# Atif-Anwer/SHMGAN

Hardware: AMD Instinct MI355X
Metric: images/sec (gen+disc train_step) (higher is better)
Workload: dtype f32; 1 GPU; SHMGAN train_step 256x256 5-view, batch 8/GPU, filter_size 64, fp32 (BASELINE configs[1]); global_batch=8, image_size=256, parallelism=dp1, losses_finite=True

## Files before the change

### include/shmgan_hip.h

```cpp
#ifndef SHMGAN_HIP_H
#define SHMGAN_HIP_H

#include <stddef.h>

#ifdef __cplusplus
extern "C" {
#endif

#define SHM_OK 0
#define SHM_E_SHAPE (-1)
#define SHM_E_DTYPE (-2)
#define SHM_E_WORKSPACE (-3)
#define SHM_E_HIP (-4)

#define SHM_F32 0
#define SHM_BF16 1
#define SHM_BF16_GF32 2

int shm_version(void);
const char* shm_last_error(void);
const char* shm_last_kernel(void);

#define SHM_TG_AUTO 0
#define SHM_TG_HALO128 1
#define SHM_TG_HALO64 2
#define SHM_TG_DMA_128x128 3
#define SHM_TG_DMA_64x128 4
#define SHM_TG_DMA_128x64 5
#define SHM_TG_DMA_256x64 6
#define SHM_TG_DMA_256x128 7
#define SHM_TG_HALO128_PH8 8
#define SHM_TG_DMA_128x128_BK32 9
#define SHM_TG_DMA_128x128_NST4 10
#define SHM_TG_HALO128_ST 12
#define SHM_TG_HALO64_ST 13
#define SHM_TG_PHASE4 14
#define SHM_TG_DMA_64x64 15
#define SHM_TG_HALO128_ST_W4 16
#define SHM_TG_WREG 11
int shm_set_tuning(const char* key, int value);
int shm_get_tuning(const char* key, int* value);

int shm_transpose_taps(const float* w, void* wt, int ntaps, int rows, int cols, int rows_pad,
                       int dtype, void* stream);
int shm_transpose_taps_multi(int count, const void* const* w, void* const* wt, const int* ntaps, const int* rows,
                             const int* cols, const int* rows_pad, int dtype, void* stream);
int shm_cast_f32(const float* src, void* dst, size_t n, int dtype, void* stream);

int shm_conv2d_fwd(const void* x, const void* x2, int c1, int ldx, int ldx2, const void* wk,
                   const float* bias, void* y, int ldy, int batch, int hi, int wi, int cin,
                   int cout, int ksize, int stride, float slope, int dtype, void* stream);

#define SHM_STATS_SLOTS 16
int shm_conv2d_in_fwd(const void* x, const void* x2, int c1, int ldx, int ldx2, const void* wk,
                      const float* bias, void* y, int ldy, int batch, int hi, int wi, int cin,
                      int cout, int ksize, int stride, float slope, double* stats, double* scratch,
                      float eps, int dtype, void* stream);

int shm_conv2d_dgrad(const void* dy, int lddy, const void* w, void* dx, void* dx2, int n1,
                     int lddx, int lddx2, int batch, int hi, int wi, int cin, int cout,
                     int ksize, int stride, int dtype, void* stream);
// ... 219 lines not shown
```

### shmgan_amd/_lib.py

```python
from __future__ import annotations

import ctypes as C
import os
import re
import subprocess
from pathlib import Path

_HERE = Path(__file__).resolve().parent
LIB_PATH = Path(os.environ["SHM_LIB_PATH"]) if os.environ.get("SHM_LIB_PATH") else _HERE / "libshmgan_hip.so"
CSRC = _HERE / "csrc"
HEADER = _HERE.parent / "include" / "shmgan_hip.h"
SOURCES = ["runtime.hip", "conv_igemm.hip", "conv_dma.hip", "conv_halo.hip", "conv_wreg.hip", "conv_wreg_f32.hip", "conv_phase4.hip", "conv_wreg16.hip", "conv_pingpong.hip", "conv_wgrad.hip", "conv_wgrad_gen.hip", "conv_wgrad_halo.hip", "conv_wgrad_halo16.hip", "conv_wgrad_halo8.hip", "conv_wgrad_x3.hip", "conv_fwd_x3.hip", "conv_rgb.hip", "elem.hip", "instnorm.hip", "instnorm_bwd.hip", "instnorm_bwd_2pass.hip", "instnorm_bwd_fused8.hip", "instnorm_bwd_fusedg.hip", "grad_sums.hip", "heads.hip", "dgrad_sum1.hip", "color.hip", "imgloss.hip", "metrics.hip", "specseg.hip", "data.hip", "polar.hip", "export.hip", "telemetry.hip"]
SHARED_HEADERS = [CSRC / "common.h", CSRC / "elem.h", CSRC / "ablate.h", CSRC / "tapgemm.h", CSRC / "tapgemm_dev.h", CSRC / "wgrad.h", CSRC / "in_bwd.h", CSRC / "x3split.h", HEADER]
F32, BF16 = 0, 1
HIPCC_FLAGS = ["--offload-arch=gfx950", "-O3", "-fPIC", "-shared", "-munsafe-fp-atomics",
               "-Wall", "-Wno-unused-function", "-Wno-unused-local-typedef"]

EXTRA_FLAGS = {"conv_pingpong.hip": ["-fno-slp-vectorize"]}

P, I, Z, F = C.c_void_p, C.c_int, C.c_size_t, C.c_float

SIGNATURES = {
    "shm_version": (I, []),
    "shm_last_error": (C.c_char_p, []),
    "shm_last_kernel": (C.c_char_p, []),
    "shm_set_tuning": (I, [C.c_char_p, I]),
    "shm_get_tuning": (I, [C.c_char_p, P]),
    "shm_transpose_taps": (I, [P, P, I, I, I, I, I, P]),
    "shm_transpose_taps_multi": (I, [I, P, P, P, P, P, P, I, P]),
    "shm_cast_f32": (I, [P, P, Z, I, P]),
    "shm_conv2d_fwd": (I, [P, P, I, I, I, P, P, P, I, I, I, I, I, I, I, I, F, I, P]),
    "shm_conv2d_in_fwd": (I, [P, P, I, I, I, P, P, P, I, I, I, I, I, I, I, I, F, P, P, F, I, P]),
    "shm_conv2d_dgrad": (I, [P, I, P, P, P, I, I, I, I, I, I, I, I, I, I, I, P]),
    "shm_conv2d_transpose_fwd": (I, [P, I, P, P, P, I, I, I, I, I, I, F, I, P]),
    "shm_conv2d_wgrad_workspace": (Z, [I, I, I, I, I, I]),
# ... 151 lines not shown
```

### shmgan_amd/csrc/common.h

```cpp
#pragma once
#include <hip/hip_runtime.h>
#include <stddef.h>
#include <stdint.h>
#include <stdio.h>

#include "../../include/shmgan_hip.h"

typedef float f32x4 __attribute__((ext_vector_type(4)));
typedef float f32x16 __attribute__((ext_vector_type(16)));

typedef __bf16 bf16_t;

void shm_set_error(const char* fmt, ...);
void shm_set_last_kernel(const char* fmt, ...);

int shm_rgb_s2_fwd_launch(const void* x, int ldx, const void* wk, int K, const float* bias, void* y, int ldy, int batch, int hi, int wi, int cout, float slope,
                          double* stats, int stats_slots, unsigned stats_stride, size_t xbytes, size_t ybytes, int dtype, hipStream_t st);
int shm_rgb_s2_wgrad_launch(const void* x, int ldx, const void* dy, int lddy, float* part, size_t ws_bytes, int batch, int hi, int wi, int cin, int cout,
                            size_t xbytes, size_t dybytes, int dtype, int* nsplit_out, hipStream_t st);

int shm_in_finalize_internal(double* stats, double* part, int nslot, int total, int hw, double eps, float* nt, const float* beta, int c, hipStream_t st);
int shm_gsum_reduce_internal(const void* g, int ldg, const void* aux, int ldaux, double* red, int batch, int hw, int c, int dtype, hipStream_t st);

enum ShmTune {
// ... 2 lines not shown
    SHM_TUNE_TAPGEMM_SMALL_GRID,
    SHM_TUNE_TAPGEMM_PHASE4_MIN,
    SHM_TUNE_WGRAD_VARIANT,
    SHM_TUNE_WGRAD_BLOCKS,
    SHM_TUNE_WGRAD_BF16_ROWS,
    SHM_TUNE_STATS_FUSION,
    SHM_TUNE_ELEM_REVERSE,
    SHM_TUNE_ELEM_REDUCE_BLOCKS,
    SHM_TUNE_ELEM_NT,
    SHM_TUNE_ELEM_CHUNK_MB,
    SHM_TUNE_ELEM_INTERLEAVE,
    SHM_TUNE_ELEM_STREAM_BLOCKS,
    SHM_TUNE_ELEM_APPLY_BLOCKS,
    SHM_TUNE_TAPGEMM_WREG16,
    SHM_TUNE_WGRAD_BF16_WIDE,
    SHM_TUNE_WGRAD_F32_SPLIT,
    SHM_TUNE_TAPGEMM_FLAT_EPILOGUE,
    SHM_TUNE_ELEM_FUSED_BWD,
    SHM_TUNE_ELEM_FUSED_MAX_SLICES,
    SHM_TUNE_CONV_F32_SPLIT,
    SHM_TUNE_ELEM_FUSED_TEST_STALL,
    SHM_TUNE_ELEM_FUSED_HOLD,
    SHM_TUNE_ELEM_FUSED_GVARIANT,
    SHM_TUNE_COUNT
};
int shm_tune(int id);
unsigned long long* shm_clock_probe();

#define SHM_LDS_BARRIER()                                       \
    do {                                                        \
        asm volatile("s_waitcnt lgkmcnt(0)" ::: "memory");      \
        __builtin_amdgcn_s_barrier();                           \
    } while (0)

typedef unsigned shm_u32x4 __attribute__((ext_vector_type(4)));
__device__ __forceinline__ shm_u32x4 shm_rsrc_words(const void* p, unsigned bytes) {
    const unsigned long long a = (unsigned long long)p;
    return shm_u32x4{(unsigned)a, (unsigned)(a >> 32) & 0xffffu, bytes, 0x00020000u};
}
__device__ __forceinline__ void shm_dma16(const shm_u32x4 rs, const unsigned lds_addr, const unsigned voff) {
    unsigned keep;
    asm volatile("s_mov_b32 %0, m0\n\ts_mov_b32 m0, %1\n\ts_nop 0\n\tbuffer_load_dwordx4 %2, %3, 0 offen lds\n\ts_mov_b32 m0, %0"
                 : "=&s"(keep)
                 : "s"(lds_addr), "v"(voff), "s"(rs)
                 : "memory");
}
__device__ __forceinline__ unsigned shm_lds_addr(const void* p) {
    return (unsigned)(size_t)(__attribute__((address_space(3))) const void*)p;
}

#define SHM_TG_COUNT 17

__device__ __forceinline__ f32x4 ld4(const float* p) { return *(const f32x4*)p; }
__device__ __forceinline__ f32x4 ld4(const bf16_t* p) {
    const uint2 u = *(const uint2*)p;
    f32x4 r;
    r[0] = __uint_as_float(u.x << 16);
    r[1] = __uint_as_float(u.x & 0xffff0000u);
    r[2] = __uint_as_float(u.y << 16);
    r[3] = __uint_as_float(u.y & 0xffff0000u);
    return r;
}
__device__ __forceinline__ f32x4 ld4nt(const float* p) { return __builtin_nontemporal_load((const f32x4*)p); }
__device__ __forceinline__ f32x4 ld4nt(const bf16_t* p) {
    typedef unsigned u32x2_t __attribute__((ext_vector_type(2)));
    const u32x2_t u = __builtin_nontemporal_load((const u32x2_t*)p);
    f32x4 r;
    r[0] = __uint_as_float(u[0] << 16);
    r[1] = __uint_as_float(u[0] & 0xffff0000u);
    r[2] = __uint_as_float(u[1] << 16);
    r[3] = __uint_as_float(u[1] & 0xffff0000u);
    return r;
}
__device__ __forceinline__ void st4(float* p, f32x4 v) { *(f32x4*)p = v; }
// ... 121 lines not shown
```

### shmgan_amd/csrc/conv_halo.hip

```cpp
#include "tapgemm_dev.h"

template <typename T, typename TO, int BN, int PH = 16, bool ST = false, int TM = 2, bool GS = false, int NM = 0>
__global__ __launch_bounds__(BN * PH / (2 * TM), ST ? BN * PH / (256 * TM) : 1) void tapgemm_halo_kernel(const TapGemmArgs a) {
    static_assert(TM == 2 || (TM == 4 && ST), "four M tiles per wave: static-tap form only");
    static_assert(!NM || (ST && TM == 2 && !GS), "norm: static-tap forward form");
    constexpr int ESZ = sizeof(T), CHE = 16 / ESZ, BKE = 64 / ESZ;
    constexpr int WGM = PH / (2 * TM), WGN = BN / 64, NW = WGM * WGN;
    constexpr int HC = 18, NIT = PH == 16 ? 24 : 12;
    constexpr int NHR = NIT * 16;
    constexpr int ASTG = NHR * 16, BSTG = BN * 16;
    constexpr int NA = NIT / NW, NB = (BN / 16) / NW;
    static_assert(NIT % NW == 0 && (BN / 16) % NW == 0, "DMA items divide over the waves");
    __shared__ __attribute__((aligned(1024))) float smem[2 * ASTG + 3 * BSTG];
    __shared__ __attribute__((aligned(1024))) float snt[NM ? SHM_NT_PLANES * SHM_NT_MAXC : 4];
    float* const sA = smem;
    float* const sB = smem + 2 * ASTG;
    typedef __attribute__((address_space(3))) void* lds_ptr;

    const TapPhase& P = a.ph[0];
    const int tid = threadIdx.x;
    const int lane = tid & 63, wave = __builtin_amdgcn_readfirstlane(tid >> 6);
    const int l31 = lane & 31, h = lane >> 5;
    const int wm = wave / WGN, wn = wave % WGN;
    const int ppr = a.wi >> 4, ppi = (a.hi / PH) * ppr;
// ... 458 lines not shown
            const int py = 2 * TM * wm + 2 * i + (row >> 4), px = row & 15;
            const size_t opix = ((size_t)img * a.hi + (y0 + py)) * a.wi + (x0 + px);
#pragma unroll
            for (int j = 0; j < 2; ++j) {
                const int n = n0 + wn * 64 + j * 32 + l31;
                if (n < a.nout) {
                    float v = acc[i][j][r] + bj[j];
                    const TO vo = (TO)shm_lrelu(v, a.slope);
                    v = (float)vo;
                    s1[j] += v;
                    s2[j] = __builtin_fmaf(v, v, s2[j]);
                    if (!abl::nostore || v == 123.456f)
                    {
                        if (n < a.n1)
                            ((TO*)a.y)[opix * a.ldy + n] = vo;
                        else
                            ((TO*)a.y2)[opix * a.ldy2 + (n - a.n1)] = vo;
                    }
                }
            }
        }
    }
    }
    if (a.stats) {
        const int slot = (prem * WGM + wm) % a.stats_slots;
#pragma unroll
        for (int j = 0; j < 2; ++j) {
            float t1 = s1[j] + __shfl_xor(s1[j], 32, 64);
            float t2 = s2[j] + __shfl_xor(s2[j], 32, 64);
            const int n = n0 + wn * 64 + j * 32 + l31;
            if (h == 0 && n < a.nout) {
                double* dst = a.stats + (size_t)slot * a.stats_stride + ((size_t)img * a.nout + n) * 2;
                atomicAdd(dst, (double)t1);
                atomicAdd(dst + 1, (double)t2);
            }
        }
    }
}

template <typename T, typename TO, int BN, int PH = 16, bool ST = false, int TM = 2, bool GS = false, int NM = 0>
static void halo_launch(const TapGemmArgs& a, int batch, hipStream_t st) {
    hipLaunchKernelGGL((tapgemm_halo_kernel<T, TO, BN, PH, ST, TM, GS, NM>), dim3(batch * (a.hi / PH) * (a.wi / 16), shm_cdiv(a.nout, BN), 1), dim3(BN * PH / (2 * TM)), 0, st, a);
    shm_set_last_kernel("tapgemm_halo_kernel<%s, %s, %d, %d, %s, %d%s>", shm_tg_name<T>(), shm_tg_name<TO>(), BN, PH, ST ? "true" : "false", TM,
                        NM == 2 ? ", false, 2" : NM == 1 ? ", false, 1" : GS ? ", true" : "");
}

template <typename T, typename TO, int BN>
static void halo_st_launch(const TapGemmArgs& a, const TapGemmPlan& p, int batch, hipStream_t st) {
    if (p.gs_fused)
        halo_launch<T, TO, BN, 16, true, 2, true>(a, batch, st);
    else if (a.nt) {
        if constexpr (sizeof(T) == sizeof(TO)) {
            if (a.ntmode)
                halo_launch<T, TO, BN, 16, true, 2, false, 2>(a, batch, st);
            else
                halo_launch<T, TO, BN, 16, true, 2, false, 1>(a, batch, st);
        }
    } else
        halo_launch<T, TO, BN, 16, true>(a, batch, st);
}
// ... 27 lines not shown
```

### shmgan_amd/csrc/conv_igemm.hip

```cpp
#include "tapgemm.h"

struct ConvExtras {
    double* stats = nullptr;
    int stats_hw = 0, stats_slots = 1;
    const void* gaux[2] = {};
    int ldgaux[2] = {};
    double* gred[2] = {};
    ShmNormReq norm = {};
    bool gsum_fused = false;
};

static TapGemmPlan tapgemm_plan(const TapGemmArgs& a, int batch, int nphase, int esz, int oesz, bool two_src, bool want_norm) {
    const int BKE = 64 / esz;
    const int forced = shm_tune(SHM_TUNE_TAPGEMM_VARIANT);
    bool halo_ok = nphase == 1 && a.is == 1 && a.os == 1 && a.ph[0].ntaps == 9 && a.hi % 16 == 0 && a.wi % 16 == 0 && a.hg == a.hi && a.wg == a.wi;
    if (halo_ok)
        for (int t = 0; t < 9; ++t)
            halo_ok = halo_ok && a.ph[0].dh[t] >= -1 && a.ph[0].dh[t] <= 1 && a.ph[0].dw[t] >= -1 && a.ph[0].dw[t] <= 1;
    const bool bk32_ok = a.K % (2 * BKE) == 0 && (!two_src || a.c1 % (2 * BKE) == 0);
    const bool wreg_ok = esz == 2 && halo_ok && !two_src && (a.K == 32 || a.K == 64) && a.ybytes != 0 && (a.y2 == nullptr || a.y2bytes != 0) &&
                         a.slope >= 0.f && a.slope <= 1.f &&
                         (oesz == 4 || (a.nout % 64 == 0 && a.n1 % 32 == 0 && a.ldy % 8 == 0 && ((size_t)a.y & 15) == 0 &&
                                        (a.y2 == nullptr || (a.ldy2 % 8 == 0 && ((size_t)a.y2 & 15) == 0))));
    const int wreg32_wn = a.nout % 64 == 0 ? 4 : a.nout == 32 ? 2 : a.nout == 16 ? 1 : 0;
    const bool wreg32_ok = esz == 4 && oesz == 4 && halo_ok && (!two_src || (a.c1 == 16 && a.K == 32 && a.nout == 16)) && a.ybytes != 0 &&
                           (a.y2 == nullptr || a.y2bytes != 0) && a.slope >= 0.f && a.slope <= 1.f && a.n1 % 16 == 0 &&
                           ((wreg32_wn == 4 && (a.K == 16 || a.K == 32 || a.K == 64)) || (wreg32_wn == 2 && a.hi % 16 == 0 && (a.K == 16 || a.K == 32)) ||
                            (wreg32_wn == 1 && a.hi % 32 == 0 && (a.K == 16 || a.K == 32)));
    bool phase4_ok = nphase == 4 && a.is == 1 && a.os == 2 && !two_src && a.y2 == nullptr && a.stats == nullptr && a.hi % 16 == 0 &&
                     a.wi % 16 == 0 && a.hg == a.hi && a.wg == a.wi && a.ho == 2 * a.hi && a.wo == 2 * a.wi && a.nout % 64 == 0 &&
                     a.ph[0].ntaps == 4 && a.ph[1].ntaps == 2 && a.ph[2].ntaps == 2 && a.ph[3].ntaps == 1;
    if (phase4_ok)
        for (int p = 0; p < 4; ++p)
            for (int t = 0; t < a.ph[p].ntaps; ++t)
                phase4_ok = phase4_ok && a.ph[p].dh[t] >= -1 && a.ph[p].dh[t] <= 1 && a.ph[p].dw[t] >= -1 && a.ph[p].dw[t] <= 1;
    int v = forced;
    if (v == SHM_TG_AUTO) {
        const long tiles128 = (long)shm_cdiv(a.M, 128) * shm_cdiv(a.nout, 128) * nphase;
        if (wreg_ok || wreg32_ok) {
            v = SHM_TG_WREG;
        } else if (phase4_ok && (long)batch * (a.hi / 16) * (a.wi / 16) * (a.nout / 64) >= shm_tune(SHM_TUNE_TAPGEMM_PHASE4_MIN) &&
                   (esz == 2 || a.K <= 256)) {
            v = SHM_TG_PHASE4;
        } else if (halo_ok) {
            const long np16 = (long)batch * (a.hi / 16) * (a.wi / 16);
            const long nb128 = np16 * shm_cdiv(a.nout, 128), nb64 = np16 * shm_cdiv(a.nout, 64);
            auto fill = [](long nb) { return (double)nb / (double)(((nb + 511) / 512) * 512); };
            if (esz == 4 && nb64 < 256)
                v = SHM_TG_DMA_64x64;
            else if (a.nout <= 64)
                v = SHM_TG_HALO64_ST;
            else if (esz == 4 && nb128 < shm_tune(SHM_TUNE_TAPGEMM_HALO_MIN))
                v = (double)((nb128 + 255) / 256) <= (double)((nb64 + 255) / 256) * 0.52 ? SHM_TG_HALO128_ST : SHM_TG_HALO64_ST;
            else if (nb128 >= (esz == 2 ? 512 : shm_tune(SHM_TUNE_TAPGEMM_HALO_MIN)) || fill(nb128) * 1.03 >= fill(nb64))
                v = SHM_TG_HALO128_ST;
            else
                v = SHM_TG_HALO64_ST;
        } else if ((long)shm_cdiv(a.M, 64) * shm_cdiv(a.nout, 128) * nphase < 256) {
            v = SHM_TG_DMA_64x64;
        } else if (nphase == 1 && a.nout > 64 && a.K <= (esz == 2 ? 256 : 128) &&
                   (long)shm_cdiv(a.M, 256) * shm_cdiv(a.nout, 128) >= 256) {
            v = SHM_TG_DMA_256x128;
        } else if (nphase == 1 && a.nout > 64 && bk32_ok && (esz == 2 ? a.K >= 256 : (a.K >= 256 && a.K < 512 && a.is == 2 && tiles128 >= 512))) {
            v = SHM_TG_DMA_128x128_BK32;
        } else if (a.nout > 64 && tiles128 < shm_tune(SHM_TUNE_TAPGEMM_SMALL_GRID)) {
            v = SHM_TG_DMA_64x128;
        } else if (a.nout > 64) {
            v = SHM_TG_DMA_128x128;
        } else {
            v = SHM_TG_DMA_128x64;
        }
    }
    const bool want_gs = a.gred[0] || a.gred[1];
    bool gs_fused = false;
    if (want_gs) {
        bool al = true;
        for (int p = 0; p < 2; ++p)
            if (a.gred[p]) al = al && (oesz == 4 || (a.ldgaux[p] % 8 == 0 && ((size_t)a.gaux[p] & 15) == 0));
        al = al && (a.y2 == nullptr || a.n1 % 32 == 0);
        const bool small = a.ybytes != 0 && (a.y2 == nullptr || a.y2bytes != 0);
// ... 20 lines not shown
    }
    bool norm_ok = false;
    if (want_norm) {
        const int pc = a.ntpart ? a.K - a.c1 : a.c1;
        norm_ok = !want_gs && nphase == 1 && a.ntc == pc && pc % BKE == 0 && pc <= SHM_NT_MAXC && (a.ntpart == 0 || two_src);
        switch (v) {
        case SHM_TG_HALO128_ST: case SHM_TG_HALO64_ST:
            norm_ok = norm_ok && halo_ok && oesz == esz;
            break;
        case SHM_TG_WREG:
            norm_ok = norm_ok && a.ntpart == 0 && pc <= 64 && ((wreg_ok && oesz == 2) || (wreg32_ok && wreg32_wn == 4 && !two_src));
            break;
        default:
            norm_ok = false;
        }
    }
    const bool x3 = esz == 4 && oesz == 4 && shm_tune(SHM_TUNE_CONV_F32_SPLIT) == 1 && halo_ok && (!want_norm || a.ntmode == 0) &&
                    (v == SHM_TG_HALO128_ST || v == SHM_TG_HALO64_ST || (v == SHM_TG_WREG && forced == SHM_TG_AUTO)) && (!want_gs || gs_fused) && shm_x3_fwd_eligible(a);
    const int w16 = shm_tune(SHM_TUNE_TAPGEMM_WREG16);
    int wreg16 = 0;
    if (v == SHM_TG_WREG && wreg_ok && oesz == 2 && w16 != 0 && !gs_fused && !want_norm && a.nout % 64 == 0 && (a.y2 == nullptr || a.n1 % 64 == 0) && !two_src &&
        a.ybytes != 0 && (a.y2 == nullptr || a.y2bytes != 0))
        wreg16 = w16 == 2 && shm_pp_eligible(a) ? 2 : 1;
    return TapGemmPlan{v, gs_fused, norm_ok, halo_ok, bk32_ok, wreg_ok, wreg32_ok, phase4_ok, wreg32_wn, x3, wreg16};
}

static int finish_args(TapGemmArgs& a, int batch, int nphase, int dtype, bool two_src, const char* who, const ConvExtras& ex) {
    SHM_REQUIRE(dtype == SHM_F32 || dtype == SHM_BF16 || dtype == SHM_BF16_GF32, SHM_E_DTYPE,
                "%s: dtype %d not in {SHM_F32, SHM_BF16, SHM_BF16_GF32}", who, dtype);
    a.stats = ex.stats;
    a.hw = ex.stats_hw;
    a.stats_slots = ex.stats_slots;
    a.stats_stride = (unsigned)batch * (unsigned)a.nout * 2u;
    for (int p = 0; p < 2; ++p) {
        a.gaux[p] = ex.gaux[p];
        a.ldgaux[p] = ex.ldgaux[p];
        a.gred[p] = ex.gred[p];
    }
    a.gslots = SHM_GSUM_SLOTS;
    a.gbatch = batch;
    a.nt = ex.norm.nt;
    a.ntpart = ex.norm.part;
    a.ntc = ex.norm.c;
    a.ntmode = ex.norm.mode;
    a.ntbytes = (unsigned)((size_t)batch * SHM_NT_PLANES * ex.norm.c * sizeof(float));
    a.wimg = 0;
    a.bias_img = 0;
// ... 33 lines not shown
        const bool flat = shm_tune(SHM_TUNE_TAPGEMM_FLAT_EPILOGUE) != 0;
        a.ybytes = (yb < lim && !flat) ? (unsigned)yb : 0u;
        a.y2bytes = (y2b < lim && !flat) ? (unsigned)y2b : 0u;
    }
    return SHM_OK;
}

static int device_cus() {
    static const int ncu = [] {
        int dev = 0, n = 0;
        if (hipGetDevice(&dev) != hipSuccess || hipDeviceGetAttribute(&n, hipDeviceAttributeMultiprocessorCount, dev) != hipSuccess || n <= 0) n = 256;
        return n;
    }();
    return ncu;
}

static int launch_plan(const TapGemmArgs& a, const TapGemmPlan& p, int batch, int nphase, int dtype, hipStream_t st, const char* who) {
    if (p.x3) return shm_x3_fwd_launch(a, batch, p.gs_fused, st, who);
    switch (p.variant) {
    case SHM_TG_HALO128: case SHM_TG_HALO64: case SHM_TG_HALO128_ST: case SHM_TG_HALO128_ST_W4: case SHM_TG_HALO64_ST: case SHM_TG_HALO128_PH8:
        return shm_halo_launch(a, p, batch, dtype, st, who);
    case SHM_TG_PHASE4:
        return shm_phase4_launch(a, p, batch, dtype, st, who);
    case SHM_TG_WREG: {
        SHM_REQUIRE(p.wreg_ok || p.wreg32_ok, SHM_E_SHAPE,
                    "%s: forced variant wreg needs a unit-stride 3x3 layer on a map that is a multiple of 16, slope in [0,1] and: bf16 -- one source "
                    "tensor with 32/64 channels, Cout %% 64 == 0; fp32 -- one source with 16/32/64 input channels and "
                    "Cout %% 64 == 0, or 16/32 input channels with Cout = 32 (map a multiple of 16) or 16 (map a multiple of 32; also 16 + 16 from two tensors)", who);
        const int np8 = batch * (a.hi / 8) * (a.wi / 16), ncu = device_cus();
        if (p.wreg16 == 2) return shm_pp_launch(a, batch, ncu, st, who);
        if (p.wreg16 == 1) return shm_wreg16_launch(a, np8, ncu, st, who);
        return p.wreg_ok ? shm_wreg_launch(a, p, np8, ncu, dtype, st, who) : shm_wreg_f32_launch(a, p, batch, ncu, st, who);
    }
    case SHM_TG_DMA_128x128: case SHM_TG_DMA_64x128: case SHM_TG_DMA_128x64: case SHM_TG_DMA_64x64: case SHM_TG_DMA_256x64:
    case SHM_TG_DMA_256x128: case SHM_TG_DMA_128x128_BK32: case SHM_TG_DMA_128x128_NST4:
        return shm_dma_launch(a, p, nphase, dtype, st, who);
    default:
        SHM_REQUIRE(false, SHM_E_SHAPE, "%s: unknown tapgemm.variant %d", who, p.variant);
    }
    return SHM_OK;
}

static int launch_tapgemm(TapGemmArgs& a, int batch, int nphase, int dtype, hipStream_t st, const char* who, ConvExtras& ex) {
    const bool two_src = a.x2 != nullptr;
    if (const int r = finish_args(a, batch, nphase, dtype, two_src, who, ex)) return r;
    if (a.M == 0 || a.nout == 0) return SHM_OK;
// ... 401 lines not shown
```

### shmgan_amd/csrc/runtime.hip

```cpp
#include "common.h"

#include <stdarg.h>

static thread_local char g_err[512] = "";

void shm_set_error(const char* fmt, ...) {
    va_list ap;
    va_start(ap, fmt);
    vsnprintf(g_err, sizeof(g_err), fmt, ap);
    va_end(ap);
}

static thread_local char g_kernel[128] = "";

void shm_set_last_kernel(const char* fmt, ...) {
    va_list ap;
    va_start(ap, fmt);
    vsnprintf(g_kernel, sizeof(g_kernel), fmt, ap);
    va_end(ap);
}

#include <atomic>
#include <stdlib.h>
#include <string.h>
// ... 9 lines not shown
    {"tapgemm.small_grid_blocks", "SHM_TAPGEMM_SMALLM", 1024, 0, 1 << 30},
    {"tapgemm.phase4_min_blocks", "SHM_TAPGEMM_PHASE4_MIN", 256, 0, 1 << 30},
    {"wgrad.variant", "SHM_WGRAD_VARIANT", 0, 0, 3},
    {"wgrad.blocks", "SHM_WGRAD_BLOCKS", 0, 0, 1 << 20},
    {"wgrad.bf16_rows", "SHM_WGRAD_BF16_ROWS", 0, 0, 4},
    {"stats.fusion", "SHM_STATS_FUSION", 1, 0, 1},
    {"elem.reverse", "SHM_ELEM_REVERSE", 1, 0, 1},
    {"elem.reduce_blocks", "SHM_ELEM_REDUCE_BLOCKS", 0, 0, 1 << 20},
    {"elem.nt_loads", "SHM_ELEM_NT", 0, 0, 1},
    {"elem.chunk_mb", "SHM_ELEM_CHUNK_MB", 0, 0, 1 << 20},
    {"elem.interleave", "SHM_ELEM_INTERLEAVE", 1, 0, 1},
    {"elem.stream_blocks", "SHM_ELEM_STREAM_BLOCKS", 32768, 256, 1 << 20},
    {"elem.apply_blocks", "SHM_ELEM_APPLY_BLOCKS", 4096, 256, 1 << 20},
    {"tapgemm.wreg16", "SHM_TAPGEMM_WREG16", 2, 0, 2},
    {"wgrad.bf16_wide", "SHM_WGRAD_BF16_WIDE", 0, 0, 4},
    {"wgrad.f32_split", "SHM_WGRAD_F32_SPLIT", 0, 0, 1},
    {"tapgemm.flat_epilogue", "SHM_TAPGEMM_FLAT_EPILOGUE", 0, 0, 1},
    {"elem.fused_bwd", "SHM_ELEM_FUSED_BWD", 1, 0, 1},
    {"elem.fused_max_slices", "SHM_ELEM_FUSED_MAX_SLICES", 256, 1, 512},
    {"conv.f32_split", "SHM_CONV_F32_SPLIT", 0, 0, 1},
    {"elem.fused_test_stall", "SHM_ELEM_FUSED_TEST_STALL", 0, 0, 1},
    {"elem.fused_hold", "SHM_ELEM_FUSED_HOLD", 0, 0, 2},
    {"elem.fused_gvariant", "SHM_ELEM_FUSED_GVARIANT", 0, 0, 1},
};
std::atomic<int> g_tune[SHM_TUNE_COUNT];
std::atomic<int> g_tune_init{0};
void tune_init() {
    if (g_tune_init.load(std::memory_order_acquire) == 2) return;
    int expect = 0;
    if (g_tune_init.compare_exchange_strong(expect, 1)) {
        for (int i = 0; i < SHM_TUNE_COUNT; ++i) {
            const char* e = getenv(kTune[i].env);
            int v = e ? atoi(e) : kTune[i].dflt;
            if (v < kTune[i].lo || v > kTune[i].hi) v = kTune[i].dflt;
            g_tune[i].store(v);
        }
        g_tune_init.store(2, std::memory_order_release);
    } else {
        while (g_tune_init.load(std::memory_order_acquire) != 2) {
        }
    }
}
int tune_find(const char* key) {
    if (!key) return -1;
    for (int i = 0; i < SHM_TUNE_COUNT; ++i)
        if (strcmp(key, kTune[i].key) == 0) return i;
// ... 43 lines not shown
```

### shmgan_amd/csrc/tapgemm.h

```cpp
#pragma once
#include "common.h"
#include "ablate.h"

typedef unsigned u32x4 __attribute__((ext_vector_type(4)));

struct TapPhase {
    int oph, opw, ntaps;
    int dh[9], dw[9], widx[9];
};

typedef __bf16 bf16x8 __attribute__((ext_vector_type(8)));
typedef __bf16 bf16x2_t __attribute__((ext_vector_type(2)));
typedef float f32x2 __attribute__((ext_vector_type(2)));
typedef short s16x4_t __attribute__((ext_vector_type(4)));
typedef __attribute__((address_space(3))) s16x4_t* lds_s16x4_t;

struct TapGemmArgs {
    const void* x;
    const void* x2;
    int c1, ldx, ldx2;
    const void* w;
    const float* bias;
    void* y;
    void* y2;
// ... 5 lines not shown
    int M;
    unsigned xbytes, x2bytes, wbytes;
    unsigned ybytes, y2bytes;
    double* stats;
    int hw;
    int stats_slots;
    unsigned stats_stride;
    float slope;
    const void* gaux[2];
    int ldgaux[2];
    double* gred[2];
    int gslots, gbatch;
    const float* nt;
    int ntpart, ntc, ntmode;
    unsigned ntbytes, wimg;
    int bias_img;
    TapPhase ph[4];
};

struct TapGemmPlan {
    int variant;
    bool gs_fused, norm_ok;
    bool halo_ok, bk32_ok, wreg_ok, wreg32_ok, phase4_ok;
    int wreg32_wn;
    bool x3;
    int wreg16;
};

template <typename T>
constexpr const char* shm_tg_name() { return sizeof(T) == 4 ? "float" : "__bf16"; }

int shm_dma_launch(const TapGemmArgs& a, const TapGemmPlan& p, int nphase, int dtype, hipStream_t st, const char* who);
int shm_halo_launch(const TapGemmArgs& a, const TapGemmPlan& p, int batch, int dtype, hipStream_t st, const char* who);
int shm_phase4_launch(const TapGemmArgs& a, const TapGemmPlan& p, int batch, int dtype, hipStream_t st, const char* who);
int shm_wreg_launch(const TapGemmArgs& a, const TapGemmPlan& p, int np8, int ncu, int dtype, hipStream_t st, const char* who);
int shm_wreg_f32_launch(const TapGemmArgs& a, const TapGemmPlan& p, int batch, int ncu, hipStream_t st, const char* who);

int shm_wreg16_launch(const TapGemmArgs& a, int np8, int ncu, hipStream_t st, const char* who);

int shm_x3_fwd_eligible(const TapGemmArgs& a);
int shm_x3_fwd_launch(const TapGemmArgs& a, int batch, bool gs_fused, hipStream_t st, const char* who);

int shm_pp_eligible(const TapGemmArgs& a);
int shm_pp_launch(const TapGemmArgs& a, int batch, int ncu, hipStream_t st, const char* who);
```

### shmgan_amd/csrc/tapgemm_dev.h

```cpp
#pragma once
#include "tapgemm.h"

__device__ __forceinline__ int gsum_part(const TapGemmArgs& a, int n, int& nl, int& pc) {
    const int p = n < a.n1 ? 0 : 1;
    nl = p ? n - a.n1 : n;
    pc = p ? a.nout - a.n1 : a.n1;
    return p;
}

template <typename T>
__device__ __forceinline__ float gsum_aux(const void* aux, size_t idx) {
    return (float)((const T*)aux)[idx];
}

__device__ __forceinline__ void gsum_wide_accum(const u32x4& v, const u32x4& av, float (&t1)[8], float (&t2)[8]) {
#pragma unroll
    for (int e = 0; e < 4; ++e) {
        const float v0 = __uint_as_float(v[e] << 16), v1 = __uint_as_float(v[e] & 0xffff0000u);
        const float a0 = __uint_as_float(av[e] << 16), a1 = __uint_as_float(av[e] & 0xffff0000u);
        t1[2 * e] += v0;
        t1[2 * e + 1] += v1;
        t2[2 * e] += v0 * a0;
        t2[2 * e + 1] += v1 * a1;
    }
// ... 19 lines not shown
    }
    return v[0];
}

template <int CW>
__device__ __forceinline__ void gsum_wide_flush(float (&t1)[8], float (&t2)[8], int lane, double* dst) {
#pragma unroll
    for (int e = 0; e < 8; ++e) {
#pragma unroll
        for (int o = CW; o < 64; o <<= 1) {
            t1[e] += __shfl_xor(t1[e], o, 64);
            t2[e] += __shfl_xor(t2[e], o, 64);
        }
    }
    if (lane < CW && dst) {
#pragma unroll
        for (int e = 0; e < 8; ++e) {
            atomicAdd(dst + 2 * e, (double)t1[e]);
            atomicAdd(dst + 2 * e + 1, (double)t2[e]);
        }
    }
}

template <typename T, int TM, int TN>
__device__ __forceinline__ void tap_mfma(const f32x4 (&av)[TM], const f32x4 (&bv)[TN], f32x16 (&acc)[TM][TN]) {
    if constexpr (sizeof(T) == 4) {
#pragma unroll
        for (int e = 0; e < 4; ++e)
#pragma unroll
            for (int i = 0; i < TM; ++i)
#pragma unroll
                for (int j = 0; j < TN; ++j)
                    acc[i][j] = __builtin_amdgcn_mfma_f32_32x32x2f32(av[i][e], bv[j][e], acc[i][j], 0, 0, 0);
    } else {
#pragma unroll
        for (int i = 0; i < TM; ++i)
#pragma unroll
            for (int j = 0; j < TN; ++j)
                acc[i][j] = __builtin_amdgcn_mfma_f32_32x32x16_bf16(__builtin_bit_cast(bf16x8, av[i]), __builtin_bit_cast(bf16x8, bv[j]),
                                                                   acc[i][j], 0, 0, 0);
    }
}
```

### shmgan_amd/ops.py

```python
from __future__ import annotations

import torch

from ._lib import check, lib


def _stream():
    return torch.cuda.current_stream().cuda_stream


class KernelTimer:

    def __init__(self):
        self.recs = []
        self.brecs = []

    def wrap(self, sym, flops, fn, label="", fixed=False):
        e0 = torch.cuda.Event(enable_timing=True)
        e1 = torch.cuda.Event(enable_timing=True)
        e0.record()
        fn()
        e1.record()
        if not fixed:
            k = lib().shm_last_kernel()
# ... 57 lines not shown

def _p(t):
    return 0 if t is None else t.data_ptr()


def _dt(t):
    if t.dtype == torch.bfloat16:
        return 1
    if t.dtype == torch.float32:
        return 0
    raise TypeError(f"activation tensors are float32 or bfloat16, got {t.dtype}")


def _dtg(act, grad):
    d = _dt(act)
    if d == 1 and grad is not None and grad.dtype == torch.float32:
        return 2
    if grad is not None and d != 2 and _dt(grad) != d:
        raise TypeError("gradient-signal tensors are float32, or share the activation dtype")
    return d


TAPGEMM_VARIANTS = {"auto": 0, "halo128": 1, "halo64": 2, "dma128x128": 3, "dma64x128": 4, "dma128x64": 5, "dma256x64": 6,
                    "dma256x128": 7, "halo128_ph8": 8, "dma128x128_bk32": 9, "dma128x128_nst4": 10, "wreg": 11, "halo128_st": 12, "halo64_st": 13, "phase4": 14, "dma64x64": 15, "halo128_st_w4": 16}


def set_tuning(key, value):
    if isinstance(value, str):
        value = TAPGEMM_VARIANTS[value]
    check(lib().shm_set_tuning(key.encode(), int(value)), "shm_set_tuning")


def get_tuning(key):
    import ctypes
    v = ctypes.c_int(0)
    check(lib().shm_get_tuning(key.encode(), ctypes.addressof(v)), "shm_get_tuning")
    return v.value


def last_kernel():
    k = lib().shm_last_kernel()
    return k.decode() if k else ""


def cast_f32(src, dst, n):
    check(lib().shm_cast_f32(_p(src), _p(dst), n, _dt(dst), _stream()), "shm_cast_f32")

# ... 738 lines not shown
```

Before: 69.92 images/sec.

## Add halo-tiled fp32 stride-2 3x3 forward conv kernel and auto-select it

Adds a new tap-GEMM kernel for fp32 stride-2 3x3 forward convolutions. It DMA-loads an input halo patch split into even and odd rows and columns into LDS, then reuses it across all nine taps, instead of taking the generic DMA or implicit-GEMM path. Weights stream through a three-stage LDS ring while input chunks are double-buffered. The auto selector routes eligible downsampling layers (K>=128, enough tiles) to it, and the shared stats flush is factored into a helper. The aim is less redundant global traffic for strided convs, at the cost of new LDS layout, swizzle and waitcnt logic that could be wrong or occupancy-limited.

```diff
diff --git a/include/shmgan_hip.h b/include/shmgan_hip.h
--- a/include/shmgan_hip.h
+++ b/include/shmgan_hip.h
@@ -37,6 +37,7 @@
 #define SHM_TG_PHASE4 14
 #define SHM_TG_DMA_64x64 15
 #define SHM_TG_HALO128_ST_W4 16
+#define SHM_TG_HALO_S2 17
 #define SHM_TG_WREG 11
 int shm_set_tuning(const char* key, int value);
 int shm_get_tuning(const char* key, int* value);
diff --git a/shmgan_amd/_lib.py b/shmgan_amd/_lib.py
--- a/shmgan_amd/_lib.py
+++ b/shmgan_amd/_lib.py
@@ -10,7 +10,7 @@
 LIB_PATH = Path(os.environ["SHM_LIB_PATH"]) if os.environ.get("SHM_LIB_PATH") else _HERE / "libshmgan_hip.so"
 CSRC = _HERE / "csrc"
 HEADER = _HERE.parent / "include" / "shmgan_hip.h"
-SOURCES = ["runtime.hip", "conv_igemm.hip", "conv_dma.hip", "conv_halo.hip", "conv_wreg.hip", "conv_wreg_f32.hip", "conv_phase4.hip", "conv_wreg16.hip", "conv_pingpong.hip", "conv_wgrad.hip", "conv_wgrad_gen.hip", "conv_wgrad_halo.hip", "conv_wgrad_halo16.hip", "conv_wgrad_halo8.hip", "conv_wgrad_x3.hip", "conv_fwd_x3.hip", "conv_rgb.hip", "elem.hip", "instnorm.hip", "instnorm_bwd.hip", "instnorm_bwd_2pass.hip", "instnorm_bwd_fused8.hip", "instnorm_bwd_fusedg.hip", "grad_sums.hip", "heads.hip", "dgrad_sum1.hip", "color.hip", "imgloss.hip", "metrics.hip", "specseg.hip", "data.hip", "polar.hip", "export.hip", "telemetry.hip"]
+SOURCES = ["runtime.hip", "conv_igemm.hip", "conv_dma.hip", "conv_halo.hip", "conv_wreg.hip", "conv_wreg_f32.hip", "conv_phase4.hip", "conv_halo_s2.hip", "conv_wreg16.hip", "conv_pingpong.hip", "conv_wgrad.hip", "conv_wgrad_gen.hip", "conv_wgrad_halo.hip", "conv_wgrad_halo16.hip", "conv_wgrad_halo8.hip", "conv_wgrad_x3.hip", "conv_fwd_x3.hip", "conv_rgb.hip", "elem.hip", "instnorm.hip", "instnorm_bwd.hip", "instnorm_bwd_2pass.hip", "instnorm_bwd_fused8.hip", "instnorm_bwd_fusedg.hip", "grad_sums.hip", "heads.hip", "dgrad_sum1.hip", "color.hip", "imgloss.hip", "metrics.hip", "specseg.hip", "data.hip", "polar.hip", "export.hip", "telemetry.hip"]
 SHARED_HEADERS = [CSRC / "common.h", CSRC / "elem.h", CSRC / "ablate.h", CSRC / "tapgemm.h", CSRC / "tapgemm_dev.h", CSRC / "wgrad.h", CSRC / "in_bwd.h", CSRC / "x3split.h", HEADER]
 F32, BF16 = 0, 1
 HIPCC_FLAGS = ["--offload-arch=gfx950", "-O3", "-fPIC", "-shared", "-munsafe-fp-atomics",
diff --git a/shmgan_amd/csrc/common.h b/shmgan_amd/csrc/common.h
--- a/shmgan_amd/csrc/common.h
+++ b/shmgan_amd/csrc/common.h
@@ -48,6 +48,7 @@
     SHM_TUNE_ELEM_FUSED_TEST_STALL,
     SHM_TUNE_ELEM_FUSED_HOLD,
     SHM_TUNE_ELEM_FUSED_GVARIANT,
+    SHM_TUNE_TAPGEMM_HALO_S2_ROWS,
     SHM_TUNE_COUNT
 };
 int shm_tune(int id);
@@ -75,7 +76,7 @@
     return (unsigned)(size_t)(__attribute__((address_space(3))) const void*)p;
 }
 
-#define SHM_TG_COUNT 17
+#define SHM_TG_COUNT 18
 
 __device__ __forceinline__ f32x4 ld4(const float* p) { return *(const f32x4*)p; }
 __device__ __forceinline__ f32x4 ld4(const bf16_t* p) {
diff --git a/shmgan_amd/csrc/conv_halo.hip b/shmgan_amd/csrc/conv_halo.hip
--- a/shmgan_amd/csrc/conv_halo.hip
+++ b/shmgan_amd/csrc/conv_halo.hip
@@ -504,20 +504,7 @@
         }
     }
     }
-    if (a.stats) {
-        const int slot = (prem * WGM + wm) % a.stats_slots;
-#pragma unroll
-        for (int j = 0; j < 2; ++j) {
-            float t1 = s1[j] + __shfl_xor(s1[j], 32, 64);
-            float t2 = s2[j] + __shfl_xor(s2[j], 32, 64);
-            const int n = n0 + wn * 64 + j * 32 + l31;
-            if (h == 0 && n < a.nout) {
-                double* dst = a.stats + (size_t)slot * a.stats_stride + ((size_t)img * a.nout + n) * 2;
-                atomicAdd(dst, (double)t1);
-                atomicAdd(dst + 1, (double)t2);
-            }
-        }
-    }
+    if (a.stats) tap_stats_flush(a, s1, s2, (prem * WGM + wm) % a.stats_slots, img, n0 + wn * 64, l31, h);
 }
 
 template <typename T, typename TO, int BN, int PH = 16, bool ST = false, int TM = 2, bool GS = false, int NM = 0>
diff --git a/shmgan_amd/csrc/conv_halo_s2.hip b/shmgan_amd/csrc/conv_halo_s2.hip
--- /dev/null
+++ b/shmgan_amd/csrc/conv_halo_s2.hip
@@ -0,0 +1,176 @@
+#include "tapgemm_dev.h"
+
+template <int PH>
+__global__ __launch_bounds__(PH * 32, 2) void tapgemm_halo_s2_kernel(const TapGemmArgs a) {
+    constexpr int BN = 128, HC = 33;
+    constexpr int WGM = PH / 4, WGN = 2, NW = WGM * WGN;
+    constexpr int NIT = PH == 8 ? 20 : 40;
+    static_assert(PH == 8 || PH == 16, "8 x 16 or 16 x 16 output patches");
+    static_assert(NIT % NW == 0 && NIT * 16 >= (PH + 1) * HC && (BN / 16) % NW == 0, "DMA items divide over the waves");
+    constexpr int NA = NIT / NW, NB = (BN / 16) / NW;
+    constexpr int ASTG = NIT * 256, BSTG = BN * 16;
+    __shared__ __attribute__((aligned(1024))) float smem[2 * ASTG + 3 * BSTG];
+    float* const sX = smem;
+    float* const sY = smem + ASTG;
+    float* const sB = smem + 2 * ASTG;
+    typedef __attribute__((address_space(3))) void* lds_ptr;
+
+    const TapPhase& P = a.ph[0];
+    const int tid = threadIdx.x;
+    const int lane = tid & 63, wave = __builtin_amdgcn_readfirstlane(tid >> 6);
+    const int l31 = lane & 31, h = lane >> 5;
+    const int wm = wave / WGN, wn = wave % WGN;
+    const int ppr = a.wo >> 4, ppi = (a.ho / PH) * ppr;
+    const int img = blockIdx.x / ppi, prem = blockIdx.x - img * ppi;
+    const int y0 = (prem / ppr) * PH, x0 = (prem % ppr) << 4;
+    const int n0 = blockIdx.y * BN;
+
+    const int drow = lane >> 2, dq = lane & 3;
+    unsigned xrow[NA], yrow[NA];
+#pragma unroll
+    for (int j = 0; j < NA; ++j) {
+        const int R = 16 * (wave + NW * j) + drow;
+        const int e = R / HC, c = R - e * HC;
+        const int ix = 2 * x0 + (c < 17 ? 2 * c : 2 * (c - 17) + 1);
+        const int iyx = 2 * (y0 + e), iyy = iyx + 1;
+        const unsigned coff = (unsigned)((dq ^ ((R >> 2) & 3)) * 4);
+        const bool vx = e <= PH && ix < a.wi && iyx < a.hi, vy = e < PH && ix < a.wi && iyy < a.hi;
+        xrow[j] = vx ? ((unsigned)((img * a.hi + iyx) * a.wi + ix) * (unsigned)a.ldx + coff) * 4u : 0xffffffffu;
+        yrow[j] = vy ? ((unsigned)((img * a.hi + iyy) * a.wi + ix) * (unsigned)a.ldx + coff) * 4u : 0xffffffffu;
+    }
+    unsigned wrow[NB];
+#pragma unroll
+    for (int j = 0; j < NB; ++j) {
+        const int row = (wave + NW * j) * 16 + drow;
+        const int nn = n0 + row;
+        wrow[j] = nn < a.nout ? (unsigned)(nn * a.K + (dq ^ ((row >> 2) & 3)) * 4) * 4u : 0xffffffffu;
+    }
+    const __amdgpu_buffer_rsrc_t rsx = __builtin_amdgcn_make_buffer_rsrc((void*)a.x, 0, a.xbytes, 0x00020000);
+    const __amdgpu_buffer_rsrc_t rsw = __builtin_amdgcn_make_buffer_rsrc((void*)a.w, 0, a.wbytes, 0x00020000);
+
+    const int nch = a.K >> 4;
+    auto dma_half = [&](float* stage, const unsigned (&rows)[NA], int chunk) {
+        const unsigned cb = (unsigned)chunk * 64u;
+        float* dst = stage + wave * 256;
+#pragma unroll
+        for (int j = 0; j < NA; ++j) {
+            const unsigned off = rows[j] == 0xffffffffu ? rows[j] : rows[j] + cb;
+            __builtin_amdgcn_raw_ptr_buffer_load_lds(rsx, (lds_ptr)(dst + j * NW * 256), 16, (int)off, 0, 0, 0);
+        }
+    };
+    auto dma_b_at = [&](int t_wi, int chunk2, int stage2) {
+        const unsigned wbase = (unsigned)((t_wi * a.nout) * a.K + chunk2 * 16) * 4u;
+#pragma unroll
+        for (int j = 0; j < NB; ++j) {
+            const unsigned off = wrow[j] == 0xffffffffu ? wrow[j] : wrow[j] + wbase;
+            __builtin_amdgcn_raw_ptr_buffer_load_lds(rsw, (lds_ptr)(sB + stage2 * BSTG + (wave + NW * j) * 256), 16, (int)off, 0, 0, 0);
+        }
+    };
+
+    f32x16 acc[2][2];
+#pragma unroll
+    for (int i = 0; i < 2; ++i)
+#pragma unroll
+        for (int j = 0; j < 2; ++j)
+#pragma unroll
+            for (int r = 0; r < 16; ++r) acc[i][j][r] = 0.f;
+
+    constexpr int ORD[9] = {0, 1, 2, 6, 7, 8, 3, 4, 5};
+    const int prow = (l31 >> 4) ^ (((l31 + 4) >> 3) & 1), pcol = l31 & 15;
+    int fs[9][2];
+#pragma unroll
+    for (int s = 0; s < 9; ++s) {
+        const int kh = ORD[s] / 3, kw = ORD[s] % 3;
+#pragma unroll
+        for (int i = 0; i < 2; ++i) {
+            const int py = 4 * wm + 2 * i + prow;
+            const int R = (py + (kh == 2 ? 1 : 0)) * HC + (kw == 1 ? 17 : kw >> 1) + pcol;
+            fs[s][i] = (kh == 1 ? ASTG : 0) + R * 16 + ((h ^ ((R >> 2) & 3)) << 2);
+        }
+    }
+    const int swb = (l31 >> 2) & 3;
+    const int fb0 = l31 * 16 + ((0 + h) ^ swb) * 4, fb1 = l31 * 16 + ((2 + h) ^ swb) * 4;
+    int tw[9];
+#pragma unroll
+    for (int s = 0; s < 9; ++s) tw[s] = P.widx[ORD[s]];
+
+    dma_half(sX, xrow, 0);
+    dma_b_at(tw[0], 0, 0);
+    dma_b_at(tw[1], 0, 1);
+    for (int chunk = 0; chunk < nch; ++chunk) {
+        const bool more = chunk + 1 < nch;
+#pragma unroll
+        for (int s = 0; s < 9; ++s) {
+            if (s == 8 && !more)
+                asm volatile("s_waitcnt vmcnt(0)" ::: "memory");
+            else if (s == 1 || (s == 7 && more))
+                asm volatile("s_waitcnt vmcnt(%0)" ::"n"(NA + NB) : "memory");
+            else
+                asm volatile("s_waitcnt vmcnt(%0)" ::"n"(NB) : "memory");
+            SHM_LDS_BARRIER();
+            asm volatile("" ::: "memory");
+            if (s == 0) dma_half(sY, yrow, chunk);
+            if (s == 6 && more) dma_half(sX, xrow, chunk + 1);
+            if (s < 7 || more) dma_b_at(tw[(s + 2) % 9], chunk + (s + 2) / 9, (s + 2) % 3);
+            const float* Bb = sB + (s % 3) * BSTG + wn * 64 * 16;
+#pragma unroll
+            for (int kk = 0; kk < 2; ++kk) {
+                f32x4 av[2], bv[2];
+#pragma unroll
+                for (int i = 0; i < 2; ++i) av[i] = *(const f32x4*)(smem + (fs[s][i] ^ (kk << 3)));
+#pragma unroll
+                for (int j = 0; j < 2; ++j) bv[j] = *(const f32x4*)(Bb + j * 512 + (kk ? fb1 : fb0));
+                tap_mfma<float, 2, 2>(av, bv, acc);
+            }
+            asm volatile("" ::: "memory");
+        }
+    }
+
+    float s1[2], s2[2];
+#pragma unroll
+    for (int j = 0; j < 2; ++j) s1[j] = s2[j] = 0.f;
+    const __amdgpu_buffer_rsrc_t rsy = __builtin_amdgcn_make_buffer_rsrc(a.y, 0, a.ybytes, 0x00020000);
+    const unsigned ldyb = (unsigned)a.ldy * 4u;
+#pragma unroll
+    for (int j = 0; j < 2; ++j) {
+        const int n = n0 + wn * 64 + j * 32 + l31;
+        float bj = (a.bias && n < a.nout) ? a.bias[n] : 0.f;
+        asm volatile("" : "+v"(bj));
+        if (n < a.nout) {
+#pragma unroll
+            for (int i = 0; i < 2; ++i) {
+                unsigned yo[2];
+#pragma unroll
+                for (int q = 0; q < 2; ++q)
+                    yo[q] = (unsigned)((img * a.ho + (y0 + 4 * wm + 2 * i + (q ^ h))) * a.wo + x0 + 4 * h) * ldyb + (unsigned)n * 4u;
+#pragma unroll
+                for (int r = 0; r < 16; ++r) {
+                    const int q = (r >> 3) ^ ((r >> 2) & 1);
+                    const unsigned cr = (unsigned)(8 * ((r >> 2) & 1) + (r & 3));
+                    const float v = shm_lrelu(acc[i][j][r] + bj, a.slope);
+                    s1[j] += v;
+                    s2[j] = __builtin_fmaf(v, v, s2[j]);
+                    __builtin_amdgcn_raw_buffer_store_b32(__builtin_bit_cast(unsigned, v), rsy, yo[q], cr * ldyb, 0);
+                }
+            }
+        }
+    }
+    if (a.stats) tap_stats_flush(a, s1, s2, (prem * WGM + wm) % a.stats_slots, img, n0 + wn * 64, l31, h);
+}
+
+template <int PH>
+static void halo_s2_launch(const TapGemmArgs& a, int batch, hipStream_t st) {
+    hipLaunchKernelGGL((tapgemm_halo_s2_kernel<PH>), dim3(batch * (a.ho / PH) * (a.wo / 16), shm_cdiv(a.nout, 128), 1), dim3(PH * 32), 0, st, a);
+    shm_set_last_kernel("tapgemm_halo_s2_kernel<%d>", PH);
+}
+
+int shm_halo_s2_launch(const TapGemmArgs& a, const TapGemmPlan& p, int batch, hipStream_t st, const char* who) {
+    SHM_REQUIRE(p.halo_s2_ph != 0, SHM_E_SHAPE,
+                "%s: forced variant halo/stride-2 needs an fp32 stride-2 3x3 forward product from one source, no gsum or norm request, an even map whose "
+                "output is whole 8 x 16 patches, K %% 16 == 0, Cout %% 64 == 0 and an output below 4 GiB", who);
+    if (p.halo_s2_ph == 16)
+        halo_s2_launch<16>(a, batch, st);
+    else
+        halo_s2_launch<8>(a, batch, st);
+    return SHM_OK;
+}
diff --git a/shmgan_amd/csrc/conv_igemm.hip b/shmgan_amd/csrc/conv_igemm.hip
--- a/shmgan_amd/csrc/conv_igemm.hip
+++ b/shmgan_amd/csrc/conv_igemm.hip
@@ -34,6 +34,14 @@
         for (int p = 0; p < 4; ++p)
             for (int t = 0; t < a.ph[p].ntaps; ++t)
                 phase4_ok = phase4_ok && a.ph[p].dh[t] >= -1 && a.ph[p].dh[t] <= 1 && a.ph[p].dw[t] >= -1 && a.ph[p].dw[t] <= 1;
+    int halo_s2_ph = 0;
+    if (esz == 4 && oesz == 4 && nphase == 1 && a.is == 2 && a.os == 1 && a.ph[0].ntaps == 9 && !two_src && !want_norm && !a.gred[0] && !a.gred[1] &&
+        a.y2 == nullptr && a.ybytes != 0 && a.hi % 2 == 0 && a.wi % 2 == 0 && a.ho == a.hi / 2 && a.wo == a.wi / 2 && a.hg == a.ho && a.wg == a.wo &&
+        a.ho % 8 == 0 && a.wo % 16 == 0 && a.K % 16 == 0 && a.ldx >= a.K && a.nout % 64 == 0) {
+        halo_s2_ph = shm_tune(SHM_TUNE_TAPGEMM_HALO_S2_ROWS) == 16 && a.ho % 16 == 0 ? 16 : 8;
+        for (int t = 0; t < 9; ++t)
+            if (a.ph[0].dh[t] != t / 3 || a.ph[0].dw[t] != t % 3) halo_s2_ph = 0;
+    }
     int v = forced;
     if (v == SHM_TG_AUTO) {
         const long tiles128 = (long)shm_cdiv(a.M, 128) * shm_cdiv(a.nout, 128) * nphase;
@@ -56,6 +64,8 @@
                 v = SHM_TG_HALO128_ST;
             else
                 v = SHM_TG_HALO64_ST;
+        } else if (halo_s2_ph != 0 && a.K >= 128 && (long)batch * (a.ho / 8) * (a.wo / 16) * shm_cdiv(a.nout, 128) >= 512) {
+            v = SHM_TG_HALO_S2;
         } else if ((long)shm_cdiv(a.M, 64) * shm_cdiv(a.nout, 128) * nphase < 256) {
             v = SHM_TG_DMA_64x64;
         } else if (nphase == 1 && a.nout > 64 && a.K <= (esz == 2 ? 256 : 128) &&
@@ -122,7 +132,7 @@
     if (v == SHM_TG_WREG && wreg_ok && oesz == 2 && w16 != 0 && !gs_fused && !want_norm && a.nout % 64 == 0 && (a.y2 == nullptr || a.n1 % 64 == 0) && !two_src &&
         a.ybytes != 0 && (a.y2 == nullptr || a.y2bytes != 0))
         wreg16 = w16 == 2 && shm_pp_eligible(a) ? 2 : 1;
-    return TapGemmPlan{v, gs_fused, norm_ok, halo_ok, bk32_ok, wreg_ok, wreg32_ok, phase4_ok, wreg32_wn, x3, wreg16};
+    return TapGemmPlan{v, gs_fused, norm_ok, halo_ok, bk32_ok, wreg_ok, wreg32_ok, phase4_ok, halo_s2_ph, wreg32_wn, x3, wreg16};
 }
 
 static int finish_args(TapGemmArgs& a, int batch, int nphase, int dtype, bool two_src, const char* who, const ConvExtras& ex) {
@@ -202,6 +212,8 @@
         return shm_halo_launch(a, p, batch, dtype, st, who);
     case SHM_TG_PHASE4:
         return shm_phase4_launch(a, p, batch, dtype, st, who);
+    case SHM_TG_HALO_S2:
+        return shm_halo_s2_launch(a, p, batch, st, who);
     case SHM_TG_WREG: {
         SHM_REQUIRE(p.wreg_ok || p.wreg32_ok, SHM_E_SHAPE,
                     "%s: forced variant wreg needs a unit-stride 3x3 layer on a map that is a multiple of 16, slope in [0,1] and: bf16 -- one source "
diff --git a/shmgan_amd/csrc/runtime.hip b/shmgan_amd/csrc/runtime.hip
--- a/shmgan_amd/csrc/runtime.hip
+++ b/shmgan_amd/csrc/runtime.hip
@@ -55,6 +55,7 @@
     {"elem.fused_test_stall", "SHM_ELEM_FUSED_TEST_STALL", 0, 0, 1},
     {"elem.fused_hold", "SHM_ELEM_FUSED_HOLD", 0, 0, 2},
     {"elem.fused_gvariant", "SHM_ELEM_FUSED_GVARIANT", 0, 0, 1},
+    {"tapgemm.halo_s2_rows", "SHM_TAPGEMM_HALO_S2_ROWS", 0, 0, 16},
 };
 std::atomic<int> g_tune[SHM_TUNE_COUNT];
 std::atomic<int> g_tune_init{0};
diff --git a/shmgan_amd/csrc/tapgemm.h b/shmgan_amd/csrc/tapgemm.h
--- a/shmgan_amd/csrc/tapgemm.h
+++ b/shmgan_amd/csrc/tapgemm.h
@@ -51,6 +51,7 @@
     int variant;
     bool gs_fused, norm_ok;
     bool halo_ok, bk32_ok, wreg_ok, wreg32_ok, phase4_ok;
+    int halo_s2_ph;
     int wreg32_wn;
     bool x3;
     int wreg16;
@@ -62,6 +63,7 @@
 int shm_dma_launch(const TapGemmArgs& a, const TapGemmPlan& p, int nphase, int dtype, hipStream_t st, const char* who);
 int shm_halo_launch(const TapGemmArgs& a, const TapGemmPlan& p, int batch, int dtype, hipStream_t st, const char* who);
 int shm_phase4_launch(const TapGemmArgs& a, const TapGemmPlan& p, int batch, int dtype, hipStream_t st, const char* who);
+int shm_halo_s2_launch(const TapGemmArgs& a, const TapGemmPlan& p, int batch, hipStream_t st, const char* who);
 int shm_wreg_launch(const TapGemmArgs& a, const TapGemmPlan& p, int np8, int ncu, int dtype, hipStream_t st, const char* who);
 int shm_wreg_f32_launch(const TapGemmArgs& a, const TapGemmPlan& p, int batch, int ncu, hipStream_t st, const char* who);
 
diff --git a/shmgan_amd/csrc/tapgemm_dev.h b/shmgan_amd/csrc/tapgemm_dev.h
--- a/shmgan_amd/csrc/tapgemm_dev.h
+++ b/shmgan_amd/csrc/tapgemm_dev.h
@@ -65,6 +65,20 @@
     }
 }
 
+__device__ __forceinline__ void tap_stats_flush(const TapGemmArgs& a, const float (&s1)[2], const float (&s2)[2], int slot, int img, int nb, int l31, int h) {
+#pragma unroll
+    for (int j = 0; j < 2; ++j) {
+        float t1 = s1[j] + __shfl_xor(s1[j], 32, 64);
+        float t2 = s2[j] + __shfl_xor(s2[j], 32, 64);
+        const int n = nb + j * 32 + l31;
+        if (h == 0 && n < a.nout) {
+            double* dst = a.stats + (size_t)slot * a.stats_stride + ((size_t)img * a.nout + n) * 2;
+            atomicAdd(dst, (double)t1);
+            atomicAdd(dst + 1, (double)t2);
+        }
+    }
+}
+
 template <typename T, int TM, int TN>
 __device__ __forceinline__ void tap_mfma(const f32x4 (&av)[TM], const f32x4 (&bv)[TN], f32x16 (&acc)[TM][TN]) {
     if constexpr (sizeof(T) == 4) {
diff --git a/shmgan_amd/ops.py b/shmgan_amd/ops.py
--- a/shmgan_amd/ops.py
+++ b/shmgan_amd/ops.py
@@ -103,7 +103,7 @@
 
 
 TAPGEMM_VARIANTS = {"auto": 0, "halo128": 1, "halo64": 2, "dma128x128": 3, "dma64x128": 4, "dma128x64": 5, "dma256x64": 6,
-                    "dma256x128": 7, "halo128_ph8": 8, "dma128x128_bk32": 9, "dma128x128_nst4": 10, "wreg": 11, "halo128_st": 12, "halo64_st": 13, "phase4": 14, "dma64x64": 15, "halo128_st_w4": 16}
+                    "dma256x128": 7, "halo128_ph8": 8, "dma128x128_bk32": 9, "dma128x128_nst4": 10, "wreg": 11, "halo128_st": 12, "halo64_st": 13, "phase4": 14, "dma64x64": 15, "halo128_st_w4": 16, "halo_s2": 17}
 
 
 def set_tuning(key, value):
```

Result: no change. 70.06 images/sec (median of 6 runs) (+0.2%).
